# timlawrenz/DINO-X

Hardware: AMD Instinct MI355X
Metric: training images/sec (source samples; 2 global views each) ViT-S/16 224px bs256/GPU (higher is better)
Workload: dtype bf16; 1 GPU; ViT-S/16 224x224x3 2.5D slice stacks, scale-aware, 2 views/sample, DINO+Gram loss, AdamW+EMA; per_gpu_batch=256, global_batch=256, local_crops=0, out_dim=8192, parallelism=dp1, hipgraph=False

## Files before the change

### dino-x_amd/dinox/_lib.py

```python
from __future__ import annotations

import ctypes as C
import os

import torch

_HERE = os.path.dirname(os.path.abspath(__file__))
LIB_PATH = os.environ.get("DINOX_LIB") or os.path.join(_HERE, "libdinox_hip.so")

F32, BF16, U16, I16 = 0, 1, 2, 3
FMT_HU_FLOAT, FMT_HU16_PNG, FMT_WINDOWED_FLOAT = 0, 1, 2
EUNSUPPORTED = -2
EPI_BIAS, EPI_GELU, EPI_DGELU, EPI_RESIDUAL, EPI_ACCUM, EPI_AUXGRAD = 1, 2, 4, 8, 16, 32

vp, i32, i64, f32 = C.c_void_p, C.c_int32, C.c_int64, C.c_float


class GemmArgs(C.Structure):
    _fields_ = [
        ("A", vp), ("B", vp), ("C", vp),
        ("M", i64), ("N", i64), ("K", i64),
        ("lda", i64), ("ldb", i64), ("ldc", i64),
        ("batch", i64), ("strideA", i64), ("strideB", i64), ("strideC", i64),
        ("transA", i32), ("transB", i32), ("in_dtype", i32), ("out_dtype", i32), ("epilogue", i32),
        ("alpha", f32),
        ("bias", vp), ("residual", vp), ("ldr", i64), ("aux", vp), ("ldaux", i64), ("colsum", vp), ("ws", vp),
    ]


class BlockFwdArgs(C.Structure):
    _fields_ = [
        ("V", i64), ("N", i64), ("D", i32), ("H", i32), ("heads", i32), ("train", i32), ("fuse_proj_ln", i32), ("fuse_fc2_ln", i32), ("eps", f32),
        ("x0", vp), ("xn1_in", vp), ("mean1_in", vp), ("rstd1_in", vp), ("xn1", vp), ("mean1", vp), ("rstd1", vp),
        ("qkv", vp), ("o", vp), ("lse", vp), ("x1", vp), ("xn2", vp), ("mean2", vp), ("rstd2", vp), ("act", vp), ("pre", vp), ("x2", vp),
        ("next_g", vp), ("next_b", vp), ("next_eps", f32), ("next_dtype", i32), ("yn", vp), ("meann", vp), ("rstdn", vp),
        ("n1w", vp), ("n1b", vp), ("n2w", vp), ("n2b", vp), ("wqkv", vp), ("wproj", vp), ("w1", vp), ("w2", vp),
        ("bqkv", vp), ("bproj", vp), ("b1", vp), ("b2", vp),
    ]


class BlockBwdArgs(C.Structure):
    _fields_ = [
        ("V", i64), ("N", i64), ("D", i32), ("H", i32), ("heads", i32), ("fuse_ln_bwd", i32),
        ("g", vp), ("g_lowp", vp), ("g_lowp_buf", vp),
        ("x0", vp), ("x1", vp), ("xn1", vp), ("xn2", vp), ("qkv", vp), ("o", vp), ("lse", vp), ("pre", vp), ("act", vp),
        ("mean1", vp), ("rstd1", vp), ("mean2", vp), ("rstd2", vp), ("n1w", vp), ("n2w", vp),
        ("wqkv_t", vp), ("wproj_t", vp), ("w1_t", vp), ("w2_t", vp),
        ("dwqkv", vp), ("dbqkv", vp), ("dwproj", vp), ("dbproj", vp), ("dw1", vp), ("db1", vp), ("dw2", vp), ("db2", vp),
        ("dn1w", vp), ("dn1b", vp), ("dn2w", vp), ("dn2b", vp),
        ("dpre", vp), ("dxn2", vp), ("d_o", vp), ("dqkv", vp), ("dxn1", vp), ("g1", vp), ("g1_lowp", vp), ("g0_lowp", vp),
        ("attn_ws", vp), ("ln_ws", vp), ("tn_ws", vp), ("tn_ws_bytes", i64),
    ]


class BlockPlan(C.Structure):
    _fields_ = [("qkv_fused", i32), ("fuse_proj_ln", i32), ("fuse_fc2_ln", i32), ("fuse_ln_bwd", i32)]


SIGNATURES = {
    "dinox_version": (i32, []),
    "dinox_last_error": (C.c_char_p, []),
    "dinox_device_ok": (i32, []),
    "dinox_gemm": (i32, [C.POINTER(GemmArgs), vp]),
    "dinox_gemm_kernel_name": (C.c_char_p, [C.POINTER(GemmArgs)]),
    "dinox_gemm_ws_bytes": (i64, [C.POINTER(GemmArgs)]),
    "dinox_colsum": (i32, [vp, vp, i64, i64, i64, i32, i32, vp]),
    "dinox_linear_residual_ln_ok": (i32, [i64, i32, i32]),
    "dinox_linear_residual_ln": (i32, [vp, vp, vp, vp, vp, vp, vp, f32, vp, i32, vp, vp, i64, i32, i32, vp]),
    "dinox_layernorm_fwd": (i32, [vp, vp, vp, vp, vp, vp, i64, i32, f32, i32, vp]),
    "dinox_layernorm_bwd_ws_bytes": (i64, [i64, i32]),
    "dinox_layernorm_bwd": (i32, [vp, vp, vp, vp, vp, vp, vp, vp, vp, vp, vp, i64, i32, i32, i32, vp]),
    "dinox_linear_ln_bwd_ok": (i32, [i64, i32, i32]),
    "dinox_linear_ln_bwd": (i32, [vp, vp, vp, vp, vp, vp, vp, vp, vp, vp, vp, vp, i64, i32, i32, i32, vp]),
    "dinox_attention_fwd": (i32, [vp, vp, vp, i32, i32, i32, i32, i32, vp]),
    "dinox_attention_bwd_ws_bytes": (i64, [i32, i32, i32]),
    "dinox_attention_bwd": (i32, [vp, vp, vp, vp, vp, vp, i32, i32, i32, i32, i32, vp]),
    "dinox_qkv_attention_ok": (i32, [i32, i32, i32, i32, i32]),
    "dinox_qkv_attention_fwd": (i32, [vp, vp, vp, vp, vp, vp, i32, i32, i32, i32, i32, vp]),
    "dinox_patch_unfold": (i32, [vp, vp, i32, i32, i32, i32, i32, vp]),
    "dinox_patch_unfold_ld": (i32, [vp, vp, i32, i32, i32, i32, i32, i32, vp]),
    "dinox_tokens_fwd": (i32, [vp, vp, vp, vp, vp, vp, i32, i32, i32, i32, i32, vp]),
    "dinox_tokens_bwd": (i32, [vp, vp, vp, vp, vp, vp, i32, i32, i32, i32, i32, vp]),
    "dinox_scale_embed_fwd": (i32, [vp] * 12 + [i32, i32, i32, f32, vp]),
    "dinox_scale_embed_bwd_ws_bytes": (i64, [i32, i32, i32]),
    "dinox_scale_embed_bwd": (i32, [vp] * 17 + [i32, i32, i32, vp]),
    "dinox_dino_ce": (i32, [vp, vp, vp, f32, f32, f32, vp, vp, vp, i32, i32, vp]),
    "dinox_dino_ce_multi": (i32, [vp, vp, vp, f32, f32, f32, vp, vp, vp, i32, i32, i32, i32, vp]),
    "dinox_colmean": (i32, [vp, vp, i32, i32, vp]),
    "dinox_center_ema": (i32, [vp, vp, f32, i32, vp]),
    "dinox_sk_ws_floats": (i64, [i32, i32]),
    "dinox_sk_col_lse": (i32, [vp, vp, f32, f32, vp, vp, i32, i32, vp]),
    "dinox_sk_row_lse": (i32, [vp, vp, f32, f32, vp, i32, i32, vp]),
    "dinox_sk_center": (i32, [vp, f32, i32, vp, vp, i32, i32, vp]),
    "dinox_gram_normalize": (i32, [vp, vp, vp, vp, vp, vp, i32, i32, i32, i32, vp]),
    "dinox_sqsum": (i32, [vp, i64, f32, vp, vp, vp]),
    "dinox_gram_normalize_bwd": (i32, [vp, vp, vp, vp, vp, i32, i32, i32, i32, i32, vp]),
    "dinox_slice_views_lds_bytes": (i64, [i32, i32]),
    "dinox_slice_views": (i32, [vp, vp, vp, vp, i32, i32, i32, vp]),
    "dinox_slice_views_patches": (i32, [vp, vp, vp, vp, i32, i32, i32, i32, i32, i32, vp]),
    "dinox_encode_preprocess_lds_bytes": (i64, [i32, i32]),
    "dinox_encode_preprocess": (i32, [vp, i32, vp, i32, vp, i32, i32, i32, C.c_double, C.c_double, i32, vp]),
    "dinox_softmax_rows": (i32, [vp, vp, i64, i32, i32, i64, vp]),
    "dinox_softmax_bwd_rows": (i32, [vp, vp, vp, f32, i64, i32, i32, i64, vp]),
    "dinox_koleo_normalize": (i32, [vp, vp, vp, vp, i64, i32, f32, vp]),
    "dinox_koleo_nn": (i32, [vp, i64, vp, vp, i32, i32, i32, i32, vp, vp, vp]),
    "dinox_koleo_loss": (i32, [vp, i32, f32, vp, vp]),
    "dinox_koleo_bwd": (i32, [vp, vp, vp, vp, i32, i32, i32, i32, f32, f32, f32, vp, vp]),
    "dinox_ntxent_rows": (i32, [vp, i64, i32, f32, vp, vp, vp, vp]),
    "dinox_ntxent_coeff": (i32, [vp, i64, vp, i32, f32, f32, vp, i64, vp]),
    "dinox_normalize_bwd": (i32, [vp, vp, vp, vp, i64, i32, f32, vp]),
    "dinox_ntxent_rows_rect": (i32, [vp, i64, i32, i32, i32, i32, f32, vp, vp, vp, vp]),
    "dinox_ntxent_coeff_rect": (i32, [vp, i64, vp, vp, i32, i32, i32, i32, f32, f32, vp, i64, vp]),
    "dinox_mae_mask_ids": (i32, [vp, vp, vp, i32, i32, i32, vp]),
    "dinox_mae_gather_unfold": (i32, [vp, vp, vp, i32, i32, i32, i32, i32, i32, i32, vp]),
    "dinox_mae_tokens_fwd": (i32, [vp, vp, vp, vp, vp, i32, i32, i32, i32, i32, vp]),
    "dinox_mae_tokens_bwd": (i32, [vp, vp, vp, vp, vp, i32, i32, i32, i32, i32, vp]),
    "dinox_mae_unshuffle_fwd": (i32, [vp, vp, vp, vp, vp, i32, i32, i32, i32, i32, vp]),
    "dinox_mae_unshuffle_bwd": (i32, [vp, vp, vp, vp, vp, vp, i32, i32, i32, i32, i32, vp]),
    "dinox_mae_loss_fwd": (i32, [vp, vp, vp, vp, vp, i32, i32, i32, i32, i32, i32, i32, vp]),
    "dinox_mae_loss_bwd": (i32, [vp, vp, vp, vp, f32, i32, i32, i32, i32, i32, i32, i32, i32, vp]),
    "dinox_ibot_put_mask": (i32, [vp, vp, vp, i32, i64, i32, i32, vp]),
    "dinox_ibot_put_mask_bwd": (i32, [vp, vp, vp, vp, i32, i64, i32, i32, vp]),
    "dinox_gather_rows": (i32, [vp, vp, vp, i64, i64, i32, i64, i32, vp]),
    "dinox_scatter_add_rows": (i32, [vp, vp, vp, i64, i64, i32, i64, i32, vp]),
    "dinox_ibot_ce": (i32, [vp, vp, vp, vp, f32, f32, f32, f32, vp, vp, vp, i32, i32, vp]),
    "dinox_ibot_center_ema": (i32, [vp, vp, f32, i32, vp]),
    "dinox_lora_down": (i32, [vp, vp, vp, i64, i32, i32, i32, i32, vp]),
    "dinox_lora_up": (i32, [vp, vp, vp, vp, f32, i64, i32, i32, i32, vp]),
    "dinox_lora_grad_ws_bytes": (i64, [i64, i32, i32, i32]),
    "dinox_lora_grad": (i32, [vp, vp, vp, vp, f32, vp, vp, vp, i64, i32, i32, i32, i32, vp]),
    "dinox_lora_dropout": (i32, [vp, vp, i64, f32, C.c_uint64, C.c_uint64, i32, vp]),
    "dinox_lora_merge": (i32, [vp, vp, vp, vp, f32, i32, i32, i32, i32, vp]),
    "dinox_seg_loss_ws_bytes": (i64, [i64, i32, i32, i32]),
    "dinox_seg_loss_fwd": (i32, [vp, vp, vp, vp, vp, vp, i64, i32, i32, i32, i32, f32, f32, vp]),
    "dinox_seg_loss_bwd": (i32, [vp, vp, vp, vp, vp, vp, i64, i32, i32, i32, i32, f32, f32, f32, vp]),
    "dinox_seg_predict": (i32, [vp, vp, vp, vp, i64, i32, i32, i32, vp]),
    "dinox_surface_ws_bytes": (i64, [i64, i32, i32, i32]),
    "dinox_surface_stats": (i32, [vp, vp, vp, vp, vp, vp, vp, vp, i64, i32, i32, i32, i32, i32, i32, vp]),
    "dinox_surface3d_ws_bytes": (i64, [i64, i32, i32, i32]),
    "dinox_surface3d_stats": (i32, [vp, vp, vp, vp, vp, vp, vp, vp, i64, i32, i32, i32, i32, i32, i32, vp]),
    "dinox_cc_ws_bytes": (i64, [i64, i32, i32, i32]),
    "dinox_cc_label": (i32, [vp, vp, vp, vp, vp, vp, vp, i64, i32, i32, i32, i32, vp]),
    "dinox_cc_filter": (i32, [vp, vp, vp, vp, vp, vp, vp, vp, i64, i32, i32, i32, i32, i32, vp]),
    "dinox_cc_match": (i32, [vp, vp, vp, vp, vp, vp, vp, vp, vp, i64, i32, i32, i32, i32, i32, vp]),
    "dinox_cc3d_ws_bytes": (i64, [i64, i32, i32, i32]),
    "dinox_cc3d_label": (i32, [vp, vp, vp, vp, vp, vp, vp, i64, i32, i32, i32, i32, vp]),
    "dinox_cc3d_filter": (i32, [vp, vp, vp, i32, vp, vp, vp, vp, i64, i32, i32, i32, i32, i32, vp]),
    "dinox_cc3d_match": (i32, [vp, vp, vp, vp, vp, vp, i32, vp, vp, i64, i32, i32, i32, i32, i32, vp]),
    "dinox_attention_rows_ok":(i32, [i32, i32, i32, i32, i32]),
    "dinox_attention_rows": (i32, [vp, vp, vp, vp, i32, i32, i32, i32, i32, i32, vp]),
    "dinox_attention_rollout_step_ok": (i32, [i32, i32, i32, i32]),
    "dinox_attention_rollout_step": (i32, [vp, vp, vp, vp, i32, i32, i32, i32, f32, i32, vp]),
    "dinox_adamw_ema": (i32, [vp, vp, vp, vp, vp, i64, f32, f32, f32, f32, f32, i32, f32, f32, vp, vp, vp]),
    "dinox_adamw_ema_dev": (i32, [vp, vp, vp, vp, vp, i64, vp, f32, f32, f32, f32, f32, f32, vp, vp, vp]),
    "dinox_sumsq": (i32, [vp, i64, vp, vp, vp]),
    "dinox_cast_bf16": (i32, [vp, vp, i64, vp]),
    "dinox_cast_transpose_bf16": (i32, [vp, vp, i32, i32, vp]),
    "dinox_cast_transpose_bf16_multi": (i32, [vp, vp, vp, i32, i64, vp]),
    "dinox_take_rows": (i32, [vp, vp, i64, i64, i32, i64, i32, vp]),
    "dinox_put_rows": (i32, [vp, vp, i64, i64, i32, i64, i32, i32, vp]),
    "dinox_axpy": (i32, [vp, vp, f32, i64, vp]),
    "dinox_lincomb3": (i32, [vp, vp, vp, f32, f32, vp, vp]),
    "dinox_zero": (i32, [vp, i64, vp]),
    "dinox_gelu_fwd": (i32, [vp, vp, i64, vp]),
    "dinox_gelu_bwd": (i32, [vp, vp, vp, i64, vp]),
    "dinox_block_plan": (i32, [i64, i64, i32, i32, i32, i32, i32, i32, C.POINTER(BlockPlan)]),
    "dinox_block_forward": (i32, [C.POINTER(BlockFwdArgs), vp]),
    "dinox_block_backward": (i32, [C.POINTER(BlockBwdArgs), vp]),
    "dinox_retrieval_ws_bytes": (i64, [i64, i64, i64]),
    "dinox_retrieval_rank": (i32, [vp, i64, vp, i64, vp, i64, i64, i64, vp, vp, vp, vp, vp, vp]),
    "dinox_retrieval_rank_windowed_ws_bytes": (i64, [i64, i64, i64]),
    "dinox_retrieval_rank_windowed": (i32, [vp, i64, vp, i64, vp, vp, vp, i64, i64, i64, vp, vp, vp, vp, vp, vp]),
    "dinox_row_dots": (i32, [vp, i64, vp, i64, i64, i64, vp, vp]),
    "dinox_knn_ws_bytes": (i64, [i64, i64, i64, i32]),
    "dinox_knn_topk": (i32, [vp, i64, vp, i64, vp, i64, i64, i64, i32, vp, vp, vp, vp]),
    "dinox_gram_ws_bytes": (i64, [i64, i64]),
    "dinox_gram_f32": (i32, [vp, i64, i64, i64, vp, vp, vp, vp, vp]),
    "dinox_softmax_probe_ws_bytes": (i64, [i64, i64, i32]),
    "dinox_softmax_probe": (i32, [vp, i64, vp, i64, i64, i32, vp, vp, vp, vp, vp, vp]),
# ... 44 lines not shown
```

### dino-x_amd/dinox/ops.py

```python
from __future__ import annotations

import contextlib
import ctypes as C
import math
import operator
import os
import weakref
from typing import Optional

import torch

from . import _lib
from ._lib import BF16, EPI_ACCUM, EPI_AUXGRAD, EPI_BIAS, EPI_DGELU, EPI_GELU, EPI_RESIDUAL, F32, BlockBwdArgs, BlockFwdArgs, BlockPlan, GemmArgs, check, lib

Tensor = torch.Tensor
_OVERRIDE: list = []


@contextlib.contextmanager
def compute_dtype(dtype: torch.dtype):
    if dtype not in (torch.float32, torch.bfloat16):
        raise ValueError("compute dtype must be torch.float32 or torch.bfloat16")
    _OVERRIDE.append(dtype)
    try:
# ... 1692 lines not shown
    check(lib.dinox_lincomb3(_p(a), _p(b), _p(c), wb, wc, _p(out), _stream()), "dinox_lincomb3")
    return out


def zero_(t: Tensor) -> None:
    assert t.is_contiguous()
    check(lib.dinox_zero(_p(t), t.numel() * t.element_size(), _stream()), "dinox_zero")


def colmean(t: Tensor) -> Tensor:
    t = _c(t.float())
    out = torch.empty(t.shape[1], dtype=torch.float32, device=t.device)
    check(lib.dinox_colmean(_p(t), _p(out), t.shape[0], t.shape[1], _stream()), "dinox_colmean")
    return out


def center_ema_(center: Tensor, batch_mean: Tensor, momentum: float) -> None:
    assert center.is_contiguous() and center.dtype == torch.float32
    check(lib.dinox_center_ema(_p(center), _p(batch_mean), momentum, center.numel(), _stream()), "dinox_center_ema")


def _sk_operand(t: Tensor) -> Tensor:
    _need_cuda(t)
    t = _c(t.float())
    assert t.dim() == 2, tuple(t.shape)
    return t


def _sk_ws(R: int, K: int, device) -> Tensor:
    return torch.empty(max(1, lib.dinox_sk_ws_floats(R, K)), dtype=torch.float32, device=device)


def sk_col_lse(t: Tensor, a: Optional[Tensor] = None, inv_temp: float = 1.0, out_scale: float = 1.0) -> Tensor:
    t = _sk_operand(t)
    R, K = t.shape
    if a is not None:
        assert a.dtype == torch.float32 and a.is_contiguous() and a.numel() == R, (tuple(a.shape), R)
    out = torch.empty(K, dtype=torch.float32, device=t.device)
    check(lib.dinox_sk_col_lse(_p(t), _p(a), inv_temp, out_scale, _p(out), _p(_sk_ws(R, K, t.device)), R, K, _stream()), "dinox_sk_col_lse")
    return out


def sk_row_lse(t: Tensor, b: Optional[Tensor] = None, inv_temp: float = 1.0, out_scale: float = 1.0) -> Tensor:
    t = _sk_operand(t)
    R, K = t.shape
    if b is not None:
        assert b.dtype == torch.float32 and b.is_contiguous() and b.numel() == K, (tuple(b.shape), K)
    out = torch.empty(R, dtype=torch.float32, device=t.device)
    check(lib.dinox_sk_row_lse(_p(t), _p(b), inv_temp, out_scale, _p(out), R, K, _stream()), "dinox_sk_row_lse")
    return out


def sk_center(t: Tensor, teacher_temp: float, n_iters: int = 3, group=None) -> Tensor:
    import torch.distributed as dist
    from .dp import exchanging
    t = _sk_operand(t)
    R, K = t.shape
    if n_iters < 1:
        raise ValueError(f"sk_center: n_iters must be >= 1, got {n_iters}")
    if not exchanging(group):
        out = torch.empty(K, dtype=torch.float32, device=t.device)
        check(lib.dinox_sk_center(_p(t), teacher_temp, n_iters, _p(out), _p(_sk_ws(R, K, t.device)), R, K, _stream()), "dinox_sk_center")
        return out
    world = dist.get_world_size(group)
    inv = C.c_float(1.0 / C.c_float(teacher_temp).value).value
    gathered = torch.empty((world, K), dtype=torch.float32, device=t.device)
    a = None
    for n in range(1, n_iters + 1):
        dist.all_gather_into_tensor(gathered, sk_col_lse(t, a, inv), group=group)
        if n == n_iters:
            return sk_col_lse(gathered, None, 1.0, teacher_temp)
        a = sk_row_lse(t, sk_col_lse(gathered, None, 1.0, -1.0), inv, -1.0)


def sk_center_idle(K: int, n_iters: int, group, device) -> None:
    import torch.distributed as dist
    world = dist.get_world_size(group)
    gathered = torch.empty((world, K), dtype=torch.float32, device=device)
    nothing = torch.full((K,), float("-inf"), dtype=torch.float32, device=device)
    for _ in range(n_iters):
        dist.all_gather_into_tensor(gathered, nothing, group=group)


def gram_loss_fwd(sf: Tensor, tf: Tensor, dt: torch.dtype):
    _need_cuda(sf, tf)
    sf, tf = _c(sf.float()), _c(tf.float())
    V, N, D = sf.shape
    T = N - 1
    dev = sf.device
    cat = torch.empty((V, T, 2 * D), dtype=dt, device=dev)
    catneg = torch.empty((V, T, 2 * D), dtype=dt, device=dev)
    shat = torch.empty((V, T, D), dtype=dt, device=dev)
    snorm = torch.empty((V, T), dtype=torch.float32, device=dev)
    check(lib.dinox_gram_normalize(_p(sf), _p(tf), _p(cat), _p(catneg), _p(shat), _p(snorm), V, N, D, _code(dt), _stream()), "dinox_gram_normalize")
    diff = gemm(cat, catneg, out_dtype=torch.float32)
    loss = torch.empty(1, dtype=torch.float32, device=dev)
    ws = torch.empty(1024, dtype=torch.float32, device=dev)
    check(lib.dinox_sqsum(_p(diff), diff.numel(), 1.0 / float(V * T * T), _p(loss), _p(ws), _stream()), "dinox_sqsum")
    return loss, (diff, shat, snorm)


def gram_loss_bwd(saved, sf_shape, scale: float, dfeats: Optional[Tensor] = None, accumulate=False) -> Tensor:
    diff, shat, snorm = saved
    V, N, D = sf_shape
    T = N - 1
    dt = shat.dtype
    d_in = diff if dt == torch.float32 else cast_bf16(diff)
    dxh = gemm(d_in, shat, transA=True, transB=True, out_dtype=torch.float32, alpha=4.0 * scale / float(V * T * T))
    if dfeats is None:
        dfeats = torch.zeros((V, N, D), dtype=torch.float32, device=diff.device)
    check(lib.dinox_gram_normalize_bwd(_p(dxh), _p(shat), _p(snorm), None, _p(dfeats), V, N, D, _code(dt), int(accumulate), _stream()),
          "dinox_gram_normalize_bwd")
    return dfeats


class GramLossFn(torch.autograd.Function):

    @staticmethod
    def forward(ctx, sf, tf):
        dt = current_dtype()
        loss, saved = gram_loss_fwd(sf, tf, dt)
        ctx.save_for_backward(*saved)
        ctx.shape = tuple(sf.shape)
        return loss.reshape(())

    @staticmethod
    def backward(ctx, g):
        d = gram_loss_bwd(ctx.saved_tensors, ctx.shape, 1.0)
        return d * g, None


def koleo_begin(x: Tensor, group=None):
    import torch.distributed as dist
    _need_cuda(x)
    x = _c(x.float())
    V, D = x.shape
    dev = x.device
    from .dp import exchanging
    gather = exchanging(group)
    world = dist.get_world_size(group) if gather else 1
    rank = dist.get_rank(group) if gather else 0
    f = lambda *sh: torch.empty(sh, dtype=torch.float32, device=dev)
    xh, norm, sq = f(V, D), f(V), f(V)
    check(lib.dinox_koleo_normalize(_p(x), _p(xh), _p(norm), _p(sq), V, D, 1e-12, _stream()), "dinox_koleo_normalize")
    works = []
    if gather:
        xh_all, sq_all = f(world * V, D), f(world * V)
        works.append(dist.all_gather_into_tensor(xh_all, xh, group=group, async_op=True))
        works.append(dist.all_gather_into_tensor(sq_all, sq, group=group, async_op=True))
    else:
        xh_all, sq_all = xh, sq
    return (xh, xh_all, sq_all, norm, works, group, gather, world, rank, V, D)


def koleo_end(state, eps: float = 1e-8):
    import torch.distributed as dist
    xh, xh_all, sq_all, norm, works, group, gather, world, rank, V, D = state
    for w in works:
        w.wait()
    dev = xh.device
    f = lambda *sh: torch.empty(sh, dtype=torch.float32, device=dev)
    Vg, row0 = world * V, rank * V
    G = gemm_nt_f32_splitk(xh, xh_all)
    idx = torch.empty(V, dtype=torch.int32, device=dev)
    dmin = f(V)
    check(lib.dinox_koleo_nn(_p(G), Vg, _p(sq_all), _p(xh_all), row0, V, Vg, D, _p(idx), _p(dmin), _stream()), "dinox_koleo_nn")
    if gather:
        idx_all = torch.empty(Vg, dtype=torch.int32, device=dev)
        d_all = f(Vg)
        dist.all_gather_into_tensor(idx_all, idx, group=group)
        dist.all_gather_into_tensor(d_all, dmin, group=group)
    else:
        idx_all, d_all = idx, dmin
    loss = f(1)
    check(lib.dinox_koleo_loss(_p(dmin), V, eps, _p(loss), _stream()), "dinox_koleo_loss")
    return loss, (xh_all, idx_all, d_all, norm, (row0, V, Vg, D), eps)


def koleo_fwd(x: Tensor, eps: float = 1e-8, group=None):
    return koleo_end(koleo_begin(x, group), eps)


def koleo_bwd(saved, gscale: float = 1.0) -> Tensor:
    xh_all, idx_all, d_all, norm, (row0, V, Vg, D), eps = saved
    dx = torch.empty((V, D), dtype=torch.float32, device=xh_all.device)
    check(lib.dinox_koleo_bwd(_p(xh_all), _p(idx_all), _p(d_all), _p(norm), row0, V, Vg, D, gscale / V, eps, 1e-12, _p(dx), _stream()),
          "dinox_koleo_bwd")
    return dx


class KoLeoFn(torch.autograd.Function):

    @staticmethod
# ... 1131 lines not shown
```

### include/dinox.h

```cpp
#ifndef DINOX_H
#define DINOX_H

#include <stddef.h>
#include <stdint.h>

#ifdef __cplusplus
extern "C" {
#endif

#define DINOX_ABI_VERSION 3

#define DINOX_F32 0
#define DINOX_BF16 1
#define DINOX_U16 2
#define DINOX_I16 3

#define DINOX_OK 0
#define DINOX_EINVAL (-1)
#define DINOX_EUNSUPPORTED (-2)
#define DINOX_EALIGN (-3)

int dinox_version(void);
const char* dinox_last_error(void);
int dinox_device_ok(void);
// ... 17 lines not shown
  int32_t in_dtype, out_dtype;
  int32_t epilogue;
  float alpha;
  const float* bias;
  const float* residual;
  int64_t ldr;
  void* aux;
  int64_t ldaux;
  float* colsum;
  void* ws;
} dinox_gemm_args;

int dinox_gemm(const dinox_gemm_args* args, void* stream);
int64_t dinox_gemm_ws_bytes(const dinox_gemm_args* args);
const char* dinox_gemm_kernel_name(const dinox_gemm_args* args);

int dinox_colsum(const void* x, float* out, int64_t M, int64_t N, int64_t ldx, int dtype, int accumulate,
                 void* stream);

int dinox_linear_residual_ln_ok(int64_t M, int N, int K);
int dinox_linear_residual_ln(const void* a, const void* w, const float* bias, const float* residual, float* x_out,
                             const float* gamma, const float* beta, float eps, void* y, int y_dtype, float* mean,
                             float* rstd, int64_t M, int N, int K, void* stream);

int dinox_layernorm_fwd(const float* x, const float* w, const float* b, void* y, float* mean, float* rstd,
                        int64_t rows, int dim, float eps, int out_dtype, void* stream);
int64_t dinox_layernorm_bwd_ws_bytes(int64_t rows, int dim);
int dinox_layernorm_bwd(const void* dy, const float* x, const float* w, const float* mean, const float* rstd,
                        float* dx, const float* dx_add, void* dx_lowp, float* dw, float* db, void* ws,
                        int64_t rows, int dim, int dy_dtype, int accumulate, void* stream);
int dinox_linear_ln_bwd_ok(int64_t M, int N, int K);
int dinox_linear_ln_bwd(const void* a, const void* w, const float* x, const float* gamma, const float* mean, const float* rstd,
                        float* dx, const float* dx_add, void* dx_lowp, float* dgamma, float* dbeta, void* ws, int64_t M, int N,
                        int K, int accumulate, void* stream);

int dinox_attention_fwd(const void* qkv, void* o, float* lse, int B, int N, int heads, int d, int dtype,
                        void* stream);
int dinox_softmax_rows(float* s, float* lse, int64_t rows, int n, int rows_per_image, int64_t lse_image_stride, void* stream);
int dinox_softmax_bwd_rows(float* s, float* dp, const float* lse, float scale, int64_t rows, int n, int rows_per_image,
                           int64_t lse_image_stride, void* stream);
int64_t dinox_attention_bwd_ws_bytes(int B, int N, int heads);
int dinox_attention_bwd(const void* d_o, const void* qkv, const void* o, const float* lse, void* dqkv, void* ws,
                        int B, int N, int heads, int d, int dtype, void* stream);
int dinox_qkv_attention_ok(int B, int N, int heads, int d, int D);
int dinox_qkv_attention_fwd(const void* x, const void* wqkv, const float* bias, void* o, void* qkv_out, float* lse, int B, int N,
                            int heads, int d, int D, void* stream);

int dinox_patch_unfold(const float* x, void* u, int V, int H, int W, int patch, int out_dtype, void* stream);
int dinox_patch_unfold_ld(const float* x, void* u, int V, int H, int W, int patch, int ld, int out_dtype, void* stream);
int dinox_tokens_fwd(const void* patches, const float* cls, const float* pos, const float* registers,
                     const float* scale, float* tokens, int V, int P, int R, int D, int patches_dtype,
                     void* stream);
int dinox_tokens_bwd(const float* dtokens, void* dpatches, float* dcls, float* dpos, float* dregs,
                     float* dscale, int V, int P, int R, int D, int patches_dtype, void* stream);

int dinox_scale_embed_fwd(const float* spacing, const float* w0, const float* b0, const float* w2,
                          const float* b2, const float* lnw, const float* lnb, float* out, float* hpre,
                          float* e, float* mean, float* rstd, int V, int h, int D, float eps, void* stream);
int64_t dinox_scale_embed_bwd_ws_bytes(int V, int h, int D);
int dinox_scale_embed_bwd(const float* dout, const float* spacing, const float* w0, const float* w2,
                          const float* lnw, const float* hpre, const float* e, const float* mean,
                          const float* rstd, float* dw0, float* db0, float* dw2, float* db2, float* dlnw,
                          float* dlnb, float* dspacing, void* ws, int V, int h, int D, void* stream);

int dinox_dino_ce(const float* s, const float* t, const float* center, float student_temp, float teacher_temp,
                  float grad_scale, float* loss, float* ds, float* row_loss, int rows2B, int K, void* stream);
int dinox_dino_ce_multi(const float* s, const float* t, const float* center, float student_temp, float teacher_temp,
                        float grad_scale, float* loss, float* ds, float* ws, int B, int n_global, int n_views, int K,
                        void* stream);
int dinox_colmean(const float* t, float* out, int rows, int K, void* stream);
int dinox_center_ema(float* center, const float* batch_mean, float momentum, int K, void* stream);

int64_t dinox_sk_ws_floats(int R, int K);
int dinox_sk_col_lse(const float* t, const float* a, float inv_temp, float out_scale, float* out, float* ws, int R, int K,
                     void* stream);
int dinox_sk_row_lse(const float* t, const float* b, float inv_temp, float out_scale, float* out, int R, int K, void* stream);
int dinox_sk_center(const float* t, float teacher_temp, int n_iters, float* center_out, float* ws, int R, int K, void* stream);

int dinox_gram_normalize(const float* sfeats, const float* tfeats, void* cat, void* catneg, void* shat,
                         float* snorm, int V, int N, int D, int out_dtype, void* stream);
int dinox_sqsum(const float* x, int64_t n, float scale, float* loss, float* ws, void* stream);
int dinox_gram_normalize_bwd(const float* dxh, const void* shat, const float* snorm, const float* sfeats,
                             float* dfeats, int V, int N, int D, int shat_dtype, int accumulate, void* stream);

int64_t dinox_slice_views_lds_bytes(int S, int max_crop);
int dinox_slice_views(const void* raw_u16, const int64_t* view_i, const float* view_f, float* out, int V, int S, int max_crop,
                      void* stream);
int dinox_slice_views_patches(const void* raw_u16, const int64_t* view_i, const float* view_f, void* u, int V, int S, int max_crop,
                              int patch, int ld, int out_dtype, void* stream);

#define DINOX_FMT_HU_FLOAT 0
#define DINOX_FMT_HU16_PNG 1
#define DINOX_FMT_WINDOWED_FLOAT 2
int64_t dinox_encode_preprocess_lds_bytes(int S, int max_side);
int dinox_encode_preprocess(const void* src, int src_dtype, const int64_t* jobs, int n_jobs, float* out, int n_images, int S,
                            int max_side, double lo, double hi, int format, void* stream);

int dinox_koleo_normalize(const float* x, float* xh, float* norm, float* sq, int64_t V, int D, float eps, void* stream);
int dinox_koleo_nn(const float* G, int64_t ldg, const float* sq_all, const float* xh_all, int row0, int V_l, int V_g, int D,
                   int* idx, float* dist, void* stream);
int dinox_koleo_loss(const float* dist, int V, float eps, float* loss, void* stream);
int dinox_koleo_bwd(const float* xh_all, const int* idx_all, const float* dist_all, const float* norm_loc, int row0, int V_l,
                    int V_g, int D, float gscale, float eps, float norm_eps, float* dx, void* stream);

int dinox_ntxent_rows(const float* S, int64_t lds, int M, float inv_tau, float* lse, float* row_loss, float* loss, void* stream);
int dinox_ntxent_coeff(const float* S, int64_t lds, const float* lse, int M, float inv_tau, float gscale, float* W, int64_t ldw,
                       void* stream);
int dinox_normalize_bwd(const float* dxh, const float* xh, const float* norm, float* dx, int64_t V, int D, float eps, void* stream);
int dinox_ntxent_rows_rect(const float* S, int64_t lds, int Ml, int Mg, int row0, int Bl, float inv_tau, float* lse, float* row_loss,
                           float* loss_sum, void* stream);
int dinox_ntxent_coeff_rect(const float* S, int64_t lds, const float* lse_local, const float* lse_all, int Ml, int Mg, int row0, int Bl,
                            float inv_tau, float gscale, float* W, int64_t ldw, void* stream);

int dinox_mae_mask_ids(const float* noise, int* ids_restore, int* ids_keep, int V, int L, int Lk, void* stream);
int dinox_mae_gather_unfold(const float* x, const int* ids_keep, void* u, int V, int H, int W, int patch, int Lk, int ld, int out_dtype,
                            void* stream);
int dinox_mae_tokens_fwd(const void* patches, const float* cls, const float* pos, const int* ids_keep, float* tokens, int V, int L, int Lk,
                         int D, int patches_dtype, void* stream);
int dinox_mae_tokens_bwd(const float* dtokens, const int* ids_restore, void* dpatches, float* dcls, float* dpos, int V, int L, int Lk, int D,
                         int patches_dtype, void* stream);
int dinox_mae_unshuffle_fwd(const void* e, const float* mask_token, const float* dec_pos, const int* ids_restore, float* xd, int V, int L,
                            int Lk, int D, int e_dtype, void* stream);
int dinox_mae_unshuffle_bwd(const float* g, const int* ids_keep, const int* ids_restore, void* de, float* dmask_token, float* ws, int V,
                            int L, int Lk, int D, int de_dtype, void* stream);
int dinox_mae_loss_fwd(const void* pred, const float* x, const int* ids_restore, float* loss, float* ws, int V, int H, int W, int patch,
                       int Lk, int lead, int pred_dtype, void* stream);
int dinox_mae_loss_bwd(const void* pred, const float* x, const int* ids_restore, void* dpred, float gscale, int V, int H, int W, int patch,
                       int Lk, int lead, int pred_dtype, int dpred_dtype, void* stream);

int dinox_ibot_put_mask(void* patches, const float* mask_token, const int* idx, int M, int64_t rows, int D, int dtype, void* stream);
int dinox_ibot_put_mask_bwd(void* dpatches, const int* idx, float* dmask_token, float* ws, int M, int64_t rows, int D, int dtype,
                            void* stream);
int dinox_gather_rows(const float* src, const int* row, void* dst, int64_t M, int64_t src_rows, int D, int64_t dst_row0, int dst_dtype,
                      void* stream);
int dinox_scatter_add_rows(const void* src, const int* row, float* dst, int64_t M, int64_t dst_rows, int D, int64_t src_row0, int src_dtype,
                           void* stream);
int dinox_ibot_ce(const float* s, const float* t, const float* center, const float* w, float student_temp, float teacher_temp, float scale,
                  float grad_scale, float* loss, float* ds, float* row_loss, int M, int K, void* stream);
int dinox_ibot_center_ema(float* center, const float* sum_count, float momentum, int K, void* stream);

int dinox_attention_rows_ok(int B, int N, int heads, int d, int Q);
int dinox_attention_rows(const void* qkv, const int* query_idx, float* probs, float* lse, int B, int N, int heads, int d, int Q, int dtype,
                         void* stream);

int dinox_attention_rollout_step_ok(int B, int N, int heads, int d);
size_t dinox_attention_rollout_step_ws_bytes(int B, int N, int heads);
int dinox_attention_rollout_step(const void* qkv, const float* w_in, float* w_out, void* ws, int B, int N, int heads, int d, float residual,
                                 int dtype, void* stream);

int dinox_adamw_ema(float* p, const float* g, float* m, float* v, float* teacher, int64_t n, float lr,
                    float weight_decay, float beta1, float beta2, float eps, int step_t, float ema,
                    float grad_scale, float* gnorm_sq, float* ws, void* stream);
int dinox_adamw_ema_dev(float* p, const float* g, float* m, float* v, float* teacher, int64_t n, const float* hyper,
                        float weight_decay, float beta1, float beta2, float eps, float ema, float grad_scale,
                        float* gnorm_sq, float* ws, void* stream);
int dinox_sumsq(const float* x, int64_t n, float* out, float* ws, void* stream);
int dinox_cast_bf16(const float* src, void* dst, int64_t n, void* stream);
int dinox_cast_transpose_bf16(const float* src, void* dst, int R, int C, void* stream);
int dinox_cast_transpose_bf16_multi(const float* src_base, void* dst_base, const int64_t* table, int n_mats,
                                    int64_t total_tiles, void* stream);
int dinox_take_rows(const float* src, void* dst, int64_t V, int64_t src_stride, int D, int64_t dst_row0, int dst_dtype,
                    void* stream);
int dinox_put_rows(const void* src, float* dst, int64_t V, int64_t dst_stride, int D, int64_t src_row0, int src_dtype,
                   int accumulate, void* stream);
int dinox_axpy(float* y, const float* x, float alpha, int64_t n, void* stream);
int dinox_lincomb3(const float* a, const float* b, const float* c, float wb, float wc, float* out, void* stream);
// ... 122 lines not shown
```

Measured before the change: 7253 samples/s.

## Fuse Gram loss normalize, Gram GEMM and squared-sum into per-view MFMA kernels

```diff
diff --git a/dino-x_amd/csrc/gram_loss.hip b/dino-x_amd/csrc/gram_loss.hip
--- /dev/null
+++ b/dino-x_amd/csrc/gram_loss.hip
@@ -0,0 +1,350 @@
+#include "common.h"
+#include "knobs.h"
+
+namespace dinox {
+
+constexpr int GL_D = 384, GL_TMAX = 208, GL_ROW = GL_D * 2;
+constexpr int GL_NRB = GL_TMAX / 16;
+constexpr int GL_NCB = GL_D / 32;
+constexpr int GL_IMG = GL_TMAX * GL_ROW;
+constexpr int GL_LDS_FWD = GL_IMG + 64, GL_LDS_BWD = GL_IMG;
+constexpr int GL_RG = 5;
+
+typedef __attribute__((address_space(3))) s16x4 gl_lds_s16x4;
+
+template <bool STUDENT>
+__device__ __forceinline__ void gl_normalize_image(const float* __restrict__ src, char* img, float* __restrict__ snorm_v, int T, int wv, int lane) {
+  for (int rbase = wv; rbase < T; rbase += 8 * GL_RG) {
+    float x[GL_RG][6];
+#pragma unroll
+    for (int q = 0; q < GL_RG; ++q) {
+      const int r = rbase + 8 * q;
+      const float* xs = src + (int64_t)(r < T ? r : 0) * GL_D;
+#pragma unroll
+      for (int k = 0; k < 6; ++k) x[q][k] = xs[lane + 64 * k];
+    }
+#pragma unroll
+    for (int q = 0; q < GL_RG; ++q) {
+      const int r = rbase + 8 * q;
+      float qs = __fmul_rn(x[q][0], x[q][0]);
+#pragma unroll
+      for (int k = 1; k < 6; ++k) qs = __fmaf_rn(x[q][k], x[q][k], qs);
+      const float ns = fmaxf(sqrtf(wave_sum(qs)), 1e-12f);
+      const float is = 1.0f / ns;
+      if (r < T) {
+        if (STUDENT && lane == 0) snorm_v[r] = ns;
+        char* const row = img + r * GL_ROW;
+#pragma unroll
+        for (int k = 0; k < 6; ++k) {
+          const float a = x[q][k] * is;
+          const int d = lane + 64 * k;
+          *reinterpret_cast<bf16_t*>(row + ((((d >> 3) ^ r) & 15) << 4) + ((d >> 7) << 8) + (d & 7) * 2) = f32_to_bf16(a);
+        }
+      }
+    }
+  }
+}
+
+__global__ __launch_bounds__(512, 2) void gram_loss_fwd_kernel(const float* __restrict__ sf, const float* __restrict__ tf, bf16_t* __restrict__ shat,
+                                                               float* __restrict__ snorm, bf16_t* __restrict__ diff,
+                                                               float* __restrict__ partial, int V, int N) {
+  extern __shared__ __attribute__((aligned(16))) char smem[];
+  double* const red = reinterpret_cast<double*>(smem + GL_IMG);
+  const int lane = threadIdx.x & 63;
+  const int wv = __builtin_amdgcn_readfirstlane(threadIdx.x >> 6);
+  const int fr = lane & 15, fq = lane >> 4;
+  const int T = N - 1;
+  const bool fast = (T & 3) == 0;
+
+  int rowoff[GL_NRB];
+  bool rowok[GL_NRB];
+#pragma unroll
+  for (int j = 0; j < GL_NRB; ++j) {
+    rowok[j] = j * 16 + fr < T;
+    rowoff[j] = rowok[j] ? (j * 16 + fr) * GL_ROW : 0;
+  }
+  const int rb0 = wv, rb1 = wv + 8;
+  const bool ok0 = rb0 * 16 + fr < T, ok1 = rb1 < GL_NRB && rb1 * 16 + fr < T;
+  const int off0 = ok0 ? (rb0 * 16 + fr) * GL_ROW : 0, off1 = ok1 ? (rb1 * 16 + fr) * GL_ROW : 0;
+  const dx_u32x4 zero4 = {0u, 0u, 0u, 0u};
+
+  for (int v = blockIdx.x; v < V; v += gridDim.x) {
+    f32x4 acc[2][GL_NRB];
+#pragma unroll
+    for (int i = 0; i < 2; ++i)
+#pragma unroll
+      for (int j = 0; j < GL_NRB; ++j) acc[i][j] = f32x4{0.f, 0.f, 0.f, 0.f};
+
+    auto product = [&](unsigned flip) {
+#pragma unroll 2
+      for (int ks = 0; ks < GL_D / 32; ++ks) {
+        const int swz = (((4 * ks + fq) ^ fr) & 15) << 4, base = (ks >> 2) << 8;
+        dx_u32x4 a0 = *reinterpret_cast<const dx_u32x4*>(smem + off0 + base + swz);
+        dx_u32x4 a1 = *reinterpret_cast<const dx_u32x4*>(smem + off1 + base + swz);
+        a0 = ok0 ? a0 ^ flip : zero4;
+        a1 = ok1 ? a1 ^ flip : zero4;
+#pragma unroll
+        for (int j = 0; j < GL_NRB; ++j) {
+          dx_u32x4 b = *reinterpret_cast<const dx_u32x4*>(smem + rowoff[j] + base + swz);
+          b = rowok[j] ? b : zero4;
+          acc[0][j] = __builtin_amdgcn_mfma_f32_16x16x32_bf16(__builtin_bit_cast(bf16x8, b), __builtin_bit_cast(bf16x8, a0), acc[0][j], 0, 0, 0);
+          acc[1][j] = __builtin_amdgcn_mfma_f32_16x16x32_bf16(__builtin_bit_cast(bf16x8, b), __builtin_bit_cast(bf16x8, a1), acc[1][j], 0, 0, 0);
+        }
+      }
+    };
+
+    __syncthreads();
+    gl_normalize_image<true>(sf + ((int64_t)v * N + 1) * GL_D, smem, snorm + (int64_t)v * T, T, wv, lane);
+    __syncthreads();
+    {
+      char* const sh = reinterpret_cast<char*>(shat + (int64_t)v * T * GL_D);
+      const int npiece = T * 48;
+      for (int u = (int)threadIdx.x; u < npiece; u += 512) {
+        const int r = u / 48, c = u - r * 48;
+        const dx_u32x4 w = *reinterpret_cast<const dx_u32x4*>(smem + r * GL_ROW + ((c & 48) << 4) + (((c ^ r) & 15) << 4));
+        *reinterpret_cast<dx_u32x4*>(sh + (int64_t)u * 16) = w;
+      }
+    }
+    product(0u);
+    __syncthreads();
+    gl_normalize_image<false>(tf + ((int64_t)v * N + 1) * GL_D, smem, nullptr, T, wv, lane);
+    __syncthreads();
+    product(0x80008000u);
+
+    double sq[4] = {0.0, 0.0, 0.0, 0.0};
+    bf16_t* const dimg = diff + (int64_t)v * T * T;
+#pragma unroll
+    for (int i = 0; i < 2; ++i) {
+      const int row = (i ? rb1 : rb0) * 16 + fr;
+      const bool rok = i ? ok1 : ok0;
+#pragma unroll
+      for (int j = 0; j < GL_NRB; ++j) {
+        const f32x4 a = acc[i][j];
+#pragma unroll
+        for (int e = 0; e < 4; ++e) sq[e] = fma((double)a[e], (double)a[e], sq[e]);
+        const int col = j * 16 + fq * 4;
+        if (rok && col < T) {
+          bf16_t* const dst = dimg + (int64_t)row * T + col;
+          if (fast) {
+            dx_u32x2 pk;
+            pk[0] = (unsigned)f32_to_bf16(a[0]) | ((unsigned)f32_to_bf16(a[1]) << 16);
+            pk[1] = (unsigned)f32_to_bf16(a[2]) | ((unsigned)f32_to_bf16(a[3]) << 16);
+            *reinterpret_cast<dx_u32x2*>(dst) = pk;
+          } else {
+#pragma unroll
+            for (int e = 0; e < 4; ++e)
+              if (col + e < T) dst[e] = f32_to_bf16(a[e]);
+          }
+        }
+      }
+    }
+    double ss = (sq[0] + sq[1]) + (sq[2] + sq[3]);
+#pragma unroll
+    for (int o = 32; o > 0; o >>= 1) ss += __shfl_xor(ss, o, 64);
+    if (lane == 0) red[wv] = ss;
+    __syncthreads();
+    if (threadIdx.x == 0) partial[v] = (float)(((red[0] + red[1]) + (red[2] + red[3])) + ((red[4] + red[5]) + (red[6] + red[7])));
+  }
+}
+
+__global__ __launch_bounds__(64) void gram_loss_sum_kernel(const float* __restrict__ partial, int n, float scale, float* __restrict__ loss) {
+  double a = 0.0;
+  for (int i = threadIdx.x; i < n; i += 64) a += (double)partial[i];
+#pragma unroll
+  for (int o = 32; o > 0; o >>= 1) a += __shfl_xor(a, o, 64);
+  if (threadIdx.x == 0) loss[0] = (float)a * scale;
+}
+
+__device__ __forceinline__ int gl_bwd_swz(int u) { return (u & 3) << 1; }
+
+__global__ __launch_bounds__(512, 2) void gram_loss_bwd_kernel(const bf16_t* __restrict__ diff, const bf16_t* __restrict__ shat,
+                                                               const float* __restrict__ snorm, float* __restrict__ dfeats, float alpha,
+                                                               int V, int N, int accumulate) {
+  extern __shared__ __attribute__((aligned(16))) char smem[];
+  const int lane = threadIdx.x & 63;
+  const int wv = __builtin_amdgcn_readfirstlane(threadIdx.x >> 6);
+  const int T = N - 1;
+  const bool fast = (T & 3) == 0;
+  const int nks = (T + 15) >> 4;
+  const int zr = 16 * nks;
+  const dx_u32x4 zero4 = {0u, 0u, 0u, 0u};
+  const int lc = lane & 31, lh = lane >> 5;
+  const int tq = (lane & 15) >> 2, tp = lane & 3, tg = (lane >> 4) & 1;
+
+  for (int v = blockIdx.x; v < V; v += gridDim.x) {
+    __syncthreads();
+    {
+      const char* const sh = reinterpret_cast<const char*>(shat + (int64_t)v * T * GL_D);
+      const int npiece = T * 48;
+      for (int u0 = (int)threadIdx.x; u0 < npiece; u0 += 4 * 512) {
+        dx_u32x4 w[4];
+#pragma unroll
+        for (int q = 0; q < 4; ++q) {
+          const int u = u0 + q * 512;
+          w[q] = u < npiece ? *reinterpret_cast<const dx_u32x4*>(sh + (int64_t)u * 16) : zero4;
+        }
+#pragma unroll
+        for (int q = 0; q < 4; ++q) {
+          const int u = u0 + q * 512;
+          const int r = u / 48, c = u - r * 48;
+          if (u < npiece) *reinterpret_cast<dx_u32x4*>(smem + r * GL_ROW + (((c >> 1) ^ gl_bwd_swz(r)) << 5) + ((c & 1) << 4)) = w[q];
+        }
+      }
+      for (int u = npiece + (int)threadIdx.x; u < zr * 48; u += 512) *reinterpret_cast<dx_u32x4*>(smem + (int64_t)u * 16) = zero4;
+    }
+    __syncthreads();
+    if (wv * 32 >= T) continue;
+
+    const bf16_t* const dimg = diff + (int64_t)v * T * T;
+    auto load_a = [&](int ks) -> dx_u32x4 {
+      const int t = wv * 32 + lc, u = ks * 16 + lh * 8;
+      dx_u32x4 r = zero4;
+      if (t < T) {
+        const bf16_t* const p = dimg + (int64_t)t * T + u;
+        if (fast) {
+          if (u < T) {
+            const dx_u32x2 lo = *reinterpret_cast<const dx_u32x2*>(p);
+            r[0] = lo[0]; r[1] = lo[1];
+          }
+          if (u + 4 < T) {
+            const dx_u32x2 hi = *reinterpret_cast<const dx_u32x2*>(p + 4);
+            r[2] = hi[0]; r[3] = hi[1];
+          }
+        } else {
+          unsigned h[8];
+#pragma unroll
+          for (int e = 0; e < 8; ++e) h[e] = u + e < T ? (unsigned)p[e] : 0u;
+          r[0] = h[0] | (h[1] << 16); r[1] = h[2] | (h[3] << 16); r[2] = h[4] | (h[5] << 16); r[3] = h[6] | (h[7] << 16);
+        }
+      }
+      return r;
+    };
+
+    f32x16 acc[GL_NCB / 2];
+    auto product = [&](const int cb0) {
+#pragma unroll
+      for (int j = 0; j < GL_NCB / 2; ++j)
+#pragma unroll
+        for (int e = 0; e < 16; ++e) acc[j][e] = 0.f;
+      dx_u32x4 an = load_a(0);
+      for (int ks = 0; ks < nks; ++ks) {
+        const dx_u32x4 a = an;
+        if (ks + 1 < nks) an = load_a(ks + 1);
+        const int k0 = ks * 16 + lh * 8 + tq, k1 = k0 + 4;
+        const int o0 = k0 * GL_ROW + 8 * tp, o1 = k1 * GL_ROW + 8 * tp;
+        const int x0 = gl_bwd_swz(k0), x1 = gl_bwd_swz(k1);
+#pragma unroll
+        for (int j = 0; j < GL_NCB / 2; ++j) {
+          const int cb = cb0 + j;
+          const s16x4 lo = __builtin_amdgcn_ds_read_tr16_b64_v4i16((gl_lds_s16x4*)(smem + o0 + (((2 * cb + tg) ^ x0) << 5)));
+          const s16x4 hi = __builtin_amdgcn_ds_read_tr16_b64_v4i16((gl_lds_s16x4*)(smem + o1 + (((2 * cb + tg) ^ x1) << 5)));
+          s16x8 b;
+          b[0] = lo[0]; b[1] = lo[1]; b[2] = lo[2]; b[3] = lo[3];
+          b[4] = hi[0]; b[5] = hi[1]; b[6] = hi[2]; b[7] = hi[3];
+          acc[j] = __builtin_amdgcn_mfma_f32_32x32x16_bf16(__builtin_bit_cast(bf16x8, a), __builtin_bit_cast(bf16x8, b), acc[j], 0, 0, 0);
+        }
+      }
+    };
+    auto s_at = [&](int tt, int cb) -> float {
+      return bf16_to_f32(*reinterpret_cast<const bf16_t*>(smem + tt * GL_ROW + (((2 * cb + (lc >> 4)) ^ gl_bwd_swz(tt)) << 5) + (lc & 15) * 2));
+    };
+    auto row_of = [&](int e) { return wv * 32 + (e & 3) + 8 * (e >> 2) + 4 * lh; };
+    float ch[16][2];
+    auto chains = [&](const int cb0) {
+#pragma unroll
+      for (int e = 0; e < 16; ++e) {
+        __builtin_amdgcn_sched_barrier(0);
+        int z;
+        asm volatile("v_mov_b32 %0, 0" : "=v"(z));
+        const int t = row_of(e), tt = t < T ? t : 0;
+#pragma unroll
+        for (int j = 0; j < GL_NCB / 2; ++j) {
+          const float g = __fmaf_rn(acc[j][e], alpha, 0.f);
+          const float sv = s_at(tt + z, cb0 + j);
+          ch[e][j & 1] = cb0 + j < 2 ? __fmaf_rn(sv, g, 0.f) : __fmaf_rn(sv, g, ch[e][j & 1]);
+        }
+      }
+    };
+    float proj[16];
+    auto output = [&](const int cb0) {
+#pragma unroll
+      for (int e = 0; e < 16; ++e) {
+        __builtin_amdgcn_sched_barrier(0);
+        int z;
+        asm volatile("v_mov_b32 %0, 0" : "=v"(z));
+        const int t = row_of(e);
+        if (t < T) {
+          const float nrm = snorm[(int64_t)v * T + t];
+          const bool clamped = !(nrm > 1e-12f);
+          const float inv = 1.0f / nrm;
+          float* const dst = dfeats + ((int64_t)v * N + 1 + t) * GL_D + lc;
+#pragma unroll
+          for (int j = 0; j < GL_NCB / 2; ++j) {
+            const int cb = cb0 + j;
+            const float g = __fmaf_rn(acc[j][e], alpha, 0.f);
+            float o = clamped ? g * 1e12f : (g - s_at(t + z, cb) * proj[e]) * inv;
+            if (accumulate) dst[cb * 32] = __fadd_rn(o, dst[cb * 32]);
+            else __builtin_nontemporal_store(o, dst + cb * 32);
+          }
+        }
+      }
+    };
+
+    product(0);
+    chains(0);
+    product(GL_NCB / 2);
+    chains(GL_NCB / 2);
+#pragma unroll
+    for (int e = 0; e < 16; ++e) {
+      float pr = ch[e][0] + ch[e][1];
+#pragma unroll
+      for (int o = 16; o > 0; o >>= 1) pr += __shfl_xor(pr, o, 64);
+      proj[e] = pr;
+    }
+#pragma unroll
+    for (int j = 0; j < GL_NCB / 2; ++j) asm volatile("" : "+v"(acc[j]) : : "memory");
+    output(GL_NCB / 2);
+    product(0);
+    output(0);
+  }
+}
+
+static bool gl_envelope(int N, int D, int dtype) { return dtype == DINOX_BF16 && D == GL_D && N >= 2 && N - 1 <= GL_TMAX; }
+static bool gl_al16(const void* p) { return (((uintptr_t)p) & 15) == 0; }
+
+}
+
+using namespace dinox;
+
+extern "C" int dinox_gram_loss_fused(int N, int D, int dtype) {
+  return gl_envelope(N, D, dtype) && knob_int("DINOX_GRAM_FUSED", 1) != 0 ? 1 : 0;
+}
+
+extern "C" int dinox_gram_loss_fwd(const float* sfeats, const float* tfeats, void* shat, float* snorm, void* diff, float* partial,
+                                   float* loss, int V, int N, int D, void* stream) {
+  DX_REQUIRE(sfeats && tfeats && shat && snorm && diff && partial && loss, DINOX_EINVAL, "gram_loss_fwd: null pointer");
+  DX_REQUIRE(V > 0 && N > 1 && D > 0, DINOX_EINVAL, "gram_loss_fwd: V=%d N=%d D=%d", V, N, D);
+  DX_REQUIRE(gl_envelope(N, D, DINOX_BF16), DINOX_EUNSUPPORTED, "gram_loss_fwd: needs D == %d and N - 1 <= %d, got N=%d D=%d", GL_D, GL_TMAX, N, D);
+  DX_REQUIRE(gl_al16(shat) && gl_al16(diff), DINOX_EINVAL, "gram_loss_fwd: shat and diff must be 16-byte aligned");
+  hipStream_t st = as_stream(stream);
+  if (int rc = reserve_lds(reinterpret_cast<const void*>(gram_loss_fwd_kernel), GL_LDS_FWD, "gram_loss_fwd")) return rc;
+  const int T = N - 1;
+  const unsigned grid = (unsigned)(V < device_cu_count() ? V : device_cu_count());
+  hipLaunchKernelGGL(gram_loss_fwd_kernel, dim3(grid), dim3(512), GL_LDS_FWD, st, sfeats, tfeats, (bf16_t*)shat, snorm, (bf16_t*)diff, partial, V, N);
+  if (int rc = check_launch("gram_loss_fwd")) return rc;
+  hipLaunchKernelGGL(gram_loss_sum_kernel, dim3(1), dim3(64), 0, st, partial, V, 1.0f / ((float)V * (float)T * (float)T), loss);
+  return check_launch("gram_loss_sum");
+}
+
+extern "C" int dinox_gram_loss_bwd(const void* diff, const void* shat, const float* snorm, float* dfeats, float alpha, int V, int N,
+                                   int D, int accumulate, void* stream) {
+  DX_REQUIRE(diff && shat && snorm && dfeats, DINOX_EINVAL, "gram_loss_bwd: null pointer");
+  DX_REQUIRE(V > 0 && N > 1 && D > 0, DINOX_EINVAL, "gram_loss_bwd: V=%d N=%d D=%d", V, N, D);
+  DX_REQUIRE(gl_envelope(N, D, DINOX_BF16), DINOX_EUNSUPPORTED, "gram_loss_bwd: needs D == %d and N - 1 <= %d, got N=%d D=%d", GL_D, GL_TMAX, N, D);
+  DX_REQUIRE(gl_al16(shat) && gl_al16(diff) && gl_al16(dfeats), DINOX_EINVAL, "gram_loss_bwd: diff, shat and dfeats must be 16-byte aligned");
+  if (int rc = reserve_lds(reinterpret_cast<const void*>(gram_loss_bwd_kernel), GL_LDS_BWD, "gram_loss_bwd")) return rc;
+  const unsigned grid = (unsigned)(V < device_cu_count() ? V : device_cu_count());
+  hipLaunchKernelGGL(gram_loss_bwd_kernel, dim3(grid), dim3(512), GL_LDS_BWD, as_stream(stream), (const bf16_t*)diff, (const bf16_t*)shat, snorm, dfeats,
+                     alpha, V, N, accumulate);
+  return check_launch("gram_loss_bwd");
+}
diff --git a/dino-x_amd/dinox/_lib.py b/dino-x_amd/dinox/_lib.py
--- a/dino-x_amd/dinox/_lib.py
+++ b/dino-x_amd/dinox/_lib.py
@@ -95,6 +95,9 @@
     "dinox_gram_normalize": (i32, [vp, vp, vp, vp, vp, vp, i32, i32, i32, i32, vp]),
     "dinox_sqsum": (i32, [vp, i64, f32, vp, vp, vp]),
     "dinox_gram_normalize_bwd": (i32, [vp, vp, vp, vp, vp, i32, i32, i32, i32, i32, vp]),
+    "dinox_gram_loss_fused": (i32, [i32, i32, i32]),
+    "dinox_gram_loss_fwd": (i32, [vp, vp, vp, vp, vp, vp, vp, i32, i32, i32, vp]),
+    "dinox_gram_loss_bwd": (i32, [vp, vp, vp, vp, f32, i32, i32, i32, i32, vp]),
     "dinox_slice_views_lds_bytes": (i64, [i32, i32]),
     "dinox_slice_views": (i32, [vp, vp, vp, vp, i32, i32, i32, vp]),
     "dinox_slice_views_patches": (i32, [vp, vp, vp, vp, i32, i32, i32, i32, i32, i32, vp]),
diff --git a/dino-x_amd/dinox/ops.py b/dino-x_amd/dinox/ops.py
--- a/dino-x_amd/dinox/ops.py
+++ b/dino-x_amd/dinox/ops.py
@@ -1798,19 +1798,29 @@
         dist.all_gather_into_tensor(gathered, nothing, group=group)
 
 
+def gram_loss_fused(N: int, D: int, dt: torch.dtype) -> bool:
+    return bool(lib.dinox_gram_loss_fused(N, D, _code(dt)))
+
+
 def gram_loss_fwd(sf: Tensor, tf: Tensor, dt: torch.dtype):
     _need_cuda(sf, tf)
     sf, tf = _c(sf.float()), _c(tf.float())
     V, N, D = sf.shape
     T = N - 1
     dev = sf.device
+    shat = torch.empty((V, T, D), dtype=dt, device=dev)
+    snorm = torch.empty((V, T), dtype=torch.float32, device=dev)
+    loss = torch.empty(1, dtype=torch.float32, device=dev)
+    if gram_loss_fused(N, D, dt):
+        diff = torch.empty((V, T, T), dtype=dt, device=dev)
+        partial = torch.empty(V, dtype=torch.float32, device=dev)
+        check(lib.dinox_gram_loss_fwd(_p(sf), _p(tf), _p(shat), _p(snorm), _p(diff), _p(partial), _p(loss), V, N, D, _stream()),
+              "dinox_gram_loss_fwd")
+        return loss, (diff, shat, snorm)
     cat = torch.empty((V, T, 2 * D), dtype=dt, device=dev)
     catneg = torch.empty((V, T, 2 * D), dtype=dt, device=dev)
-    shat = torch.empty((V, T, D), dtype=dt, device=dev)
-    snorm = torch.empty((V, T), dtype=torch.float32, device=dev)
     check(lib.dinox_gram_normalize(_p(sf), _p(tf), _p(cat), _p(catneg), _p(shat), _p(snorm), V, N, D, _code(dt), _stream()), "dinox_gram_normalize")
     diff = gemm(cat, catneg, out_dtype=torch.float32)
-    loss = torch.empty(1, dtype=torch.float32, device=dev)
     ws = torch.empty(1024, dtype=torch.float32, device=dev)
     check(lib.dinox_sqsum(_p(diff), diff.numel(), 1.0 / float(V * T * T), _p(loss), _p(ws), _stream()), "dinox_sqsum")
     return loss, (diff, shat, snorm)
@@ -1821,10 +1831,15 @@
     V, N, D = sf_shape
     T = N - 1
     dt = shat.dtype
-    d_in = diff if dt == torch.float32 else cast_bf16(diff)
-    dxh = gemm(d_in, shat, transA=True, transB=True, out_dtype=torch.float32, alpha=4.0 * scale / float(V * T * T))
+    alpha = 4.0 * scale / float(V * T * T)
     if dfeats is None:
         dfeats = torch.zeros((V, N, D), dtype=torch.float32, device=diff.device)
+    if diff.dtype == dt and gram_loss_fused(N, D, dt):
+        check(lib.dinox_gram_loss_bwd(_p(diff), _p(shat), _p(snorm), _p(dfeats), alpha, V, N, D, int(accumulate), _stream()),
+              "dinox_gram_loss_bwd")
+        return dfeats
+    d_in = diff if diff.dtype == dt else cast_bf16(diff)
+    dxh = gemm(d_in, shat, transA=True, transB=True, out_dtype=torch.float32, alpha=alpha)
     check(lib.dinox_gram_normalize_bwd(_p(dxh), _p(shat), _p(snorm), None, _p(dfeats), V, N, D, _code(dt), int(accumulate), _stream()),
           "dinox_gram_normalize_bwd")
     return dfeats
diff --git a/include/dinox.h b/include/dinox.h
--- a/include/dinox.h
+++ b/include/dinox.h
@@ -123,6 +123,11 @@
 int dinox_sqsum(const float* x, int64_t n, float scale, float* loss, float* ws, void* stream);
 int dinox_gram_normalize_bwd(const float* dxh, const void* shat, const float* snorm, const float* sfeats,
                              float* dfeats, int V, int N, int D, int shat_dtype, int accumulate, void* stream);
+int dinox_gram_loss_fused(int N, int D, int dtype);
+int dinox_gram_loss_fwd(const float* sfeats, const float* tfeats, void* shat, float* snorm, void* diff, float* partial,
+                        float* loss, int V, int N, int D, void* stream);
+int dinox_gram_loss_bwd(const void* diff, const void* shat, const float* snorm, float* dfeats, float alpha, int V, int N,
+                        int D, int accumulate, void* stream);
 
 int64_t dinox_slice_views_lds_bytes(int S, int max_crop);
 int dinox_slice_views(const void* raw_u16, const int64_t* view_i, const float* view_f, float* out, int V, int S, int max_crop,
```

Result: no change. 7296 samples/s (median of 6 runs) (+0.6%).
